# GATECH-EIC/PipeGCN

Hardware: AMD Instinct MI355X
Metric: epoch time (s), reddit 3-layer GraphSAGE (full-graph, pipelined) (lower is better)
Workload: dtype fp32; 1 GPU; model=graphsage-3L-h256, graph=reddit, num_nodes=232965, avg_degree=492, n_feat=602, n_class=41, pipeline=True, use_pp=False, norm=layer, parallelism=graph-partition dp1, num_halo=0, num_edges=114851422

## Files before the change

pipegcn_amd/csrc/bindings.cpp:

```cpp

#include "common.h"

#include <optional>

static torch::Tensor spmm(torch::Tensor indptr, torch::Tensor indices,
                          torch::Tensor feat, torch::Tensor dst_scale,
                          torch::Tensor src_scale, torch::Tensor row_order,
                          int64_t num_rows,
                          std::optional<torch::Tensor> n_live) {
  if (feat.is_cuda()) {
    auto out = torch::empty({num_rows, feat.size(1)}, feat.options());
    spmm_csr_hip(indptr, indices, feat, dst_scale, src_scale, row_order,
                 out, n_live.value_or(torch::Tensor()));
    return out;
  }
  if (feat.scalar_type() == torch::kBFloat16) {
    return spmm_cpu(indptr, indices, feat.to(torch::kFloat), dst_scale,
                    src_scale, num_rows)
        .to(torch::kBFloat16);
  }
  return spmm_cpu(indptr, indices, feat, dst_scale, src_scale, num_rows);
}

static torch::Tensor spmm_drop(torch::Tensor indptr, torch::Tensor indices,
                               torch::Tensor feat, torch::Tensor dst_scale,
                               torch::Tensor src_scale,
                               torch::Tensor row_order, int64_t num_rows,
                               bool transposed, int64_t drop_key,
                               int64_t drop_thr, double drop_scale,
                               std::optional<torch::Tensor> n_live) {
  TORCH_CHECK(feat.is_cuda() && feat.dim() == 2,
              "spmm_drop is the GPU path");
  auto out = torch::empty({num_rows, feat.size(1)}, feat.options());
  spmm_drop_hip(indptr, indices, feat, dst_scale, src_scale, row_order, out,
                n_live.value_or(torch::Tensor()), transposed, drop_key,
                drop_thr, drop_scale);
  return out;
}

static std::vector<torch::Tensor> spmm_max(torch::Tensor indptr,
                                           torch::Tensor indices,
                                           torch::Tensor z,
                                           torch::Tensor row_order,
                                           int64_t num_rows, int64_t num_cols,
                                           bool with_arg) {
  TORCH_CHECK(indptr.numel() == num_rows + 1,
              "spmm_max: indptr must hold num_rows + 1 entries");
  if (z.is_cuda())
// ... 135 lines not shown
}

static std::vector<torch::Tensor> layer_norm_relu_bwd(
    torch::Tensor dy, torch::Tensor xhat, torch::Tensor rstd,
    torch::Tensor w, torch::Tensor b, bool relu) {
  auto dx = torch::empty_like(dy);
  const int64_t N = dy.size(0);
  const int64_t F = dy.size(1);
  const int64_t nblk = std::min<int64_t>(1024, (N + 3) / 4);
  auto dw_part = torch::empty({nblk * 4, F},
                              dy.options().dtype(torch::kFloat));
  auto db_part = torch::empty_like(dw_part);
  layer_norm_relu_bwd_hip(dy.contiguous(), xhat, rstd, w, b, relu, dx,
                          dw_part, db_part);
  return {dx, colsum_hip(dw_part), colsum_hip(db_part)};
}

static void ema_update(torch::Tensor avg, torch::Tensor x, double momentum) {
  if (avg.is_cuda()) {
    ema_update_hip(avg, x, momentum);
  } else {
    avg.mul_(momentum).add_(x, 1.0 - momentum);
  }
}

PYBIND11_MODULE(TORCH_EXTENSION_NAME, m) {
  m.doc() = "pipegcn_amd native core (gfx950 HIP kernels + host graph ops)";
  m.def("build_csr", &build_csr, "COO -> CSR (counting sort by dst)");
  m.def("partition_graph", &partition_graph_cpu,
        "BFS-grown + refined k-way partitioner (cut/vol objective)");
  m.def("spmm", &spmm, "CSR SpMM with fused scale epilogue (fwd & transpose)",
        py::arg("indptr"), py::arg("indices"), py::arg("feat"),
        py::arg("dst_scale"), py::arg("src_scale"), py::arg("row_order"),
        py::arg("num_rows"), py::arg("n_live") = py::none());
  m.def("spmm_drop", &spmm_drop,
        "CSR SpMM over the edges the edge-dropout hash keeps, times "
        "drop_scale",
        py::arg("indptr"), py::arg("indices"), py::arg("feat"),
        py::arg("dst_scale"), py::arg("src_scale"), py::arg("row_order"),
        py::arg("num_rows"), py::arg("transposed"), py::arg("drop_key"),
        py::arg("drop_thr"), py::arg("drop_scale"),
        py::arg("n_live") = py::none());
  m.def("csr_simple", &csr_simple,
        "CSR without repeated entries in a row -> (indptr, indices, removed)");
  m.def("spmm_max", &spmm_max,
        "max aggregation over the CSR -> [out] or [out, arg]",
        py::arg("indptr"), py::arg("indices"), py::arg("z"),
        py::arg("row_order"), py::arg("num_rows"), py::arg("num_cols"),
        py::arg("with_arg"));
  m.def("spmm_max_bwd", &spmm_max_bwd,
        "grad_z of the max aggregation (GPU: over the simple CSC)",
        py::arg("indptr"), py::arg("indices"), py::arg("g"), py::arg("arg"),
        py::arg("row_order"), py::arg("num_src"), py::arg("num_cols"));
  m.def("scale_rows_live", &scale_rows_live,
        "g * inv per row -> (scaled, n_live = 1 + last non-zero row, int32)");
  m.def("pack_rows", &pack_rows,
        "fp32 [N, F] -> packed rows int32 [N, stride_words]");
  m.def("spmm_packed", &spmm_packed,
        "CSR SpMM over packed rows (fp32, dst_scale epilogue)");
  m.def("gather_rows", &gather_rows, "out[i,:] = src[idx[i],:]");
  m.def("gather_rows_out", &gather_rows_out,
        "gather into a preallocated out buffer");
  m.def("scatter_add_rows", &scatter_add_rows, "dst[idx[i],:] += src[i,:]");
  m.def("ema_update", &ema_update, "avg = m*avg + (1-m)*x");
  m.def("colsum", &colsum, "out[n] = sum_m x[m,n]");
  m.def("sage_dual_gemm", &sage_dual_gemm,
        "out = x1 @ w1^T + x2 @ w2^T + bias (MFMA fp32, fused)");
// ... 54 lines not shown
```

pipegcn_amd/csrc/common.h:

```cpp
#pragma once

#include <torch/extension.h>

#include <cstdint>
#include <vector>


std::vector<torch::Tensor> build_csr(torch::Tensor u, torch::Tensor v,
                                     int64_t num_rows);

torch::Tensor partition_graph_cpu(torch::Tensor indptr, torch::Tensor indices,
                                  int64_t nparts, int64_t objective,
                                  double balance_slack, int64_t n_refine_passes,
                                  int64_t seed);

torch::Tensor spmm_cpu(torch::Tensor indptr, torch::Tensor indices,
                       torch::Tensor feat, torch::Tensor dst_scale,
                       torch::Tensor src_scale, int64_t num_rows);

std::vector<torch::Tensor> max_aggregate_cpu(torch::Tensor indptr,
                                             torch::Tensor indices,
                                             torch::Tensor z, int64_t num_rows,
                                             bool with_arg);
torch::Tensor max_aggregate_bwd_cpu(torch::Tensor g, torch::Tensor arg,
                                    int64_t num_src);

std::vector<torch::Tensor> csr_simple(torch::Tensor indptr,
                                      torch::Tensor indices);


int pick_vec(int64_t F, int64_t num_rows, int64_t elem_size = 4);

std::vector<torch::Tensor> spmm_max_fwd_hip(torch::Tensor indptr,
                                            torch::Tensor indices,
                                            torch::Tensor z,
                                            torch::Tensor row_order,
                                            int64_t num_cols, bool with_arg);
torch::Tensor spmm_max_bwd_hip(torch::Tensor indptr, torch::Tensor indices,
                               torch::Tensor g, torch::Tensor arg,
                               torch::Tensor row_order, int64_t num_cols);

void spmm_csr_hip(torch::Tensor indptr, torch::Tensor indices,
                  torch::Tensor feat, torch::Tensor dst_scale,
                  torch::Tensor src_scale, torch::Tensor row_order,
                  torch::Tensor out, torch::Tensor n_live = {});

void scale_rows_live_hip(torch::Tensor g, torch::Tensor inv,
                         torch::Tensor scaled, torch::Tensor n_live);

void spmm_drop_hip(torch::Tensor indptr, torch::Tensor indices,
                   torch::Tensor feat, torch::Tensor dst_scale,
                   torch::Tensor src_scale, torch::Tensor row_order,
                   torch::Tensor out, torch::Tensor n_live, bool transposed,
                   int64_t drop_key, int64_t drop_thr, double drop_scale);

struct PackedLayout {
  int64_t mask_words;
  int64_t hdr_words;
  int64_t stride_words;
};
PackedLayout packed_layout(int64_t F);
void pack_rows_hip(torch::Tensor x, torch::Tensor packed);
void spmm_packed_hip(torch::Tensor indptr, torch::Tensor indices,
                     torch::Tensor packed, int64_t F, torch::Tensor dst_scale,
                     torch::Tensor row_order, torch::Tensor out);

void gather_rows_hip(torch::Tensor src, torch::Tensor idx, torch::Tensor out);

void scatter_add_rows_hip(torch::Tensor dst, torch::Tensor idx,
                          torch::Tensor src);

void ema_update_hip(torch::Tensor avg, torch::Tensor x, double momentum);

torch::Tensor colsum_hip(torch::Tensor x);

void dropout_fwd_hip(torch::Tensor x, torch::Tensor y, torch::Tensor mask,
                     double p, int64_t seed);
void dropout_bwd_hip(torch::Tensor dy, torch::Tensor mask, torch::Tensor dx,
// ... 53 lines not shown
```

pipegcn_amd/csrc/hip/kernels.hip:

```cpp

#include "../common.h"
#include "hip_util.h"

#include <hip/hip_bf16.h>
#include <hip/hip_runtime.h>

#include <cstdlib>
#include <vector>

namespace {

__device__ __forceinline__ void st_nt(float* p, float v) {
  __builtin_nontemporal_store(v, p);
}
__device__ __forceinline__ void st_nt(__hip_bfloat16* p, float v) {
  union {
    __hip_bfloat16 b;
    unsigned short u;
  } cv;
  cv.b = __float2bfloat16(v);
  __builtin_nontemporal_store(cv.u, reinterpret_cast<unsigned short*>(p));
}
__device__ __forceinline__ void st(float* p, float v) { *p = v; }
__device__ __forceinline__ void st(__hip_bfloat16* p, float v) {
  *p = __float2bfloat16(v);
}


template <typename T, int VEC, bool HAS_SRC_SCALE, bool HAS_LIVE>
__global__ void spmm_csr_kernel(const int64_t* __restrict__ indptr,
                                const int32_t* __restrict__ indices,
                                const T* __restrict__ feat,
                                const float* __restrict__ dst_scale,
                                const float* __restrict__ src_scale,
                                const int32_t* __restrict__ row_order,
                                T* __restrict__ out, int64_t num_rows,
                                int64_t F, int64_t nchunks,
                                const int32_t* __restrict__ n_live) {
  static_assert(!(HAS_SRC_SCALE && HAS_LIVE),
                "the redirect would also redirect the scale's index");
  int32_t live = 0;
  if constexpr (HAS_LIVE) live = max(*n_live, 0);
  auto node = [&](int32_t u) -> int64_t {
    return HAS_LIVE ? min(u, live) : u;
  };
  const int wave_in_block =
      __builtin_amdgcn_readfirstlane(static_cast<int>(threadIdx.x) / kWave);
  const int64_t waves_per_block = blockDim.x / kWave;
  const int64_t wave_global =
      static_cast<int64_t>(blockIdx.x) * waves_per_block + wave_in_block;
  const int lane = threadIdx.x & (kWave - 1);
  const int64_t nwaves = static_cast<int64_t>(gridDim.x) * waves_per_block;
  const int64_t npairs = num_rows * nchunks;

  for (int64_t pair = wave_global; pair < npairs; pair += nwaves) {
    int64_t r = pair / nchunks;
    const int64_t chunk = pair % nchunks;
    if (row_order) r = row_order[r];
    const int64_t f0 = chunk * (kWave * VEC) + lane * VEC;
    if (f0 >= F) continue;
    const bool full = (f0 + VEC <= F);

    float acc[VEC];
#pragma unroll
    for (int k = 0; k < VEC; ++k) acc[k] = 0.f;

    const int64_t e_begin = indptr[r];
    const int64_t e_end = indptr[r + 1];
    int64_t e = e_begin;

    if (full) {
// ... 13 lines not shown
        float s0 = 1.f, s1 = 1.f, s2 = 1.f, s3 = 1.f;
        if (HAS_SRC_SCALE) {
          s0 = src_scale[u0];
          s1 = src_scale[u1];
          s2 = src_scale[u2];
          s3 = src_scale[u3];
        }
        float v0[VEC], v1[VEC], v2[VEC], v3[VEC];
#pragma unroll
        for (int k = 0; k < VEC; ++k) v0[k] = to_f32(feat[u0 * F + f0 + k]);
#pragma unroll
        for (int k = 0; k < VEC; ++k) v1[k] = to_f32(feat[u1 * F + f0 + k]);
#pragma unroll
        for (int k = 0; k < VEC; ++k) v2[k] = to_f32(feat[u2 * F + f0 + k]);
#pragma unroll
        for (int k = 0; k < VEC; ++k) v3[k] = to_f32(feat[u3 * F + f0 + k]);
        if (HAS_SRC_SCALE) {
#pragma unroll
          for (int k = 0; k < VEC; ++k)
            acc[k] += s0 * v0[k] + s1 * v1[k] + s2 * v2[k] + s3 * v3[k];
        } else {
#pragma unroll
          for (int k = 0; k < VEC; ++k)
            acc[k] += v0[k] + v1[k] + v2[k] + v3[k];
        }
      }
      for (; e < e_end; ++e) {
        const int64_t u = node(indices[e]);
        const float s = HAS_SRC_SCALE ? src_scale[u] : 1.f;
#pragma unroll
        for (int k = 0; k < VEC; ++k)
          acc[k] += s * to_f32(feat[u * F + f0 + k]);
      }
      const float s = dst_scale ? dst_scale[r] : 1.f;
#pragma unroll
      for (int k = 0; k < VEC; ++k) st_nt(out + r * F + f0 + k, acc[k] * s);
    } else {
      for (; e < e_end; ++e) {
        const int64_t u = node(indices[e]);
        const float s = HAS_SRC_SCALE ? src_scale[u] : 1.f;
        for (int k = 0; k < VEC && f0 + k < F; ++k)
          acc[k] += s * to_f32(feat[u * F + f0 + k]);
      }
      const float s = dst_scale ? dst_scale[r] : 1.f;
      for (int k = 0; k < VEC && f0 + k < F; ++k)
        st(out + r * F + f0 + k, acc[k] * s);
    }
  }
}

template <typename T, int VEC>
void launch_spmm(const int64_t* indptr, const int32_t* indices,
                 const T* feat, const float* dst_scale,
                 const float* src_scale, const int32_t* row_order,
                 const int32_t* n_live, T* out, int64_t num_rows, int64_t F,
                 hipStream_t stream) {
  const int64_t nchunks = (F + kWave * VEC - 1) / (kWave * VEC);
  constexpr int threads = 256;
  static_assert(threads % kWave == 0);
  const int64_t blocks = grid_for(num_rows * nchunks, threads);
  auto launch = [&](auto kern) {
    hipLaunchKernelGGL(kern, dim3(blocks), dim3(threads), 0, stream, indptr,
                       indices, feat, dst_scale, src_scale, row_order, out,
                       num_rows, F, nchunks, n_live);
  };
  if (n_live)
    launch(HIP_KERNEL_NAME(spmm_csr_kernel<T, VEC, false, true>));
  else if (src_scale)
    launch(HIP_KERNEL_NAME(spmm_csr_kernel<T, VEC, true, false>));
  else
    launch(HIP_KERNEL_NAME(spmm_csr_kernel<T, VEC, false, false>));
  check_launch();
}


template <typename T, int VEC, bool SCATTER_ADD>
__global__ void rowcopy_kernel(const T* __restrict__ src,
                               const int64_t* __restrict__ idx,
                               T* __restrict__ dst, int64_t nrows,
                               int64_t F, int64_t nchunks) {
  const int64_t wave_global =
      (static_cast<int64_t>(blockIdx.x) * blockDim.x + threadIdx.x) / kWave;
  const int lane = threadIdx.x & (kWave - 1);
  const int64_t nwaves =
      (static_cast<int64_t>(gridDim.x) * blockDim.x) / kWave;
  const int64_t npairs = nrows * nchunks;
  for (int64_t pair = wave_global; pair < npairs; pair += nwaves) {
    const int64_t i = pair / nchunks;
    const int64_t f0 = pair % nchunks * (kWave * VEC) + lane * VEC;
    if (f0 >= F) continue;
    const int64_t j = idx[i];
    if (f0 + VEC <= F) {
#pragma unroll
      for (int k = 0; k < VEC; ++k) {
        if (SCATTER_ADD)
          st(dst + j * F + f0 + k, to_f32(dst[j * F + f0 + k]) +
                                       to_f32(src[i * F + f0 + k]));
        else
          dst[i * F + f0 + k] = src[j * F + f0 + k];
      }
    } else {
      for (int k = 0; f0 + k < F; ++k) {
        if (SCATTER_ADD)
          st(dst + j * F + f0 + k, to_f32(dst[j * F + f0 + k]) +
// ... 6 lines not shown
}

template <typename T, int VEC, bool SCATTER_ADD>
void launch_rowcopy(const T* src, const int64_t* idx, T* dst,
                    int64_t nrows, int64_t F, hipStream_t stream) {
  const int64_t nchunks = (F + kWave * VEC - 1) / (kWave * VEC);
  const int threads = 256;
  const int64_t blocks = grid_for(nrows * nchunks, threads);
  hipLaunchKernelGGL(HIP_KERNEL_NAME(rowcopy_kernel<T, VEC, SCATTER_ADD>),
                     dim3(blocks), dim3(threads), 0, stream, src, idx, dst,
                     nrows, F, nchunks);
  check_launch();
}


__global__ void ema_kernel(float* __restrict__ avg,
                           const float* __restrict__ x, float m, int64_t n) {
  const int64_t i4 = (static_cast<int64_t>(blockIdx.x) * blockDim.x +
                      threadIdx.x) * 4;
  if (i4 + 4 <= n) {
    float4 a = *reinterpret_cast<float4*>(avg + i4);
    const float4 b = *reinterpret_cast<const float4*>(x + i4);
    a.x = m * a.x + (1.f - m) * b.x;
    a.y = m * a.y + (1.f - m) * b.y;
    a.z = m * a.z + (1.f - m) * b.z;
    a.w = m * a.w + (1.f - m) * b.w;
    *reinterpret_cast<float4*>(avg + i4) = a;
  } else {
    for (int64_t i = i4; i < n; ++i) avg[i] = m * avg[i] + (1.f - m) * x[i];
  }
}


template <int VEC>
__global__ void colsum_partial_kernel(const float* __restrict__ x,
                                      float* __restrict__ partials,
                                      int64_t M, int64_t F,
                                      int64_t rows_per_blk) {
  const int64_t blk = blockIdx.x;
  const int64_t r0 = blk * rows_per_blk;
  const int64_t r1 = min(r0 + rows_per_blk, M);
  for (int64_t f0 = static_cast<int64_t>(threadIdx.x) * VEC; f0 < F;
       f0 += 256 * VEC) {
    float acc[VEC];
#pragma unroll
    for (int k = 0; k < VEC; ++k) acc[k] = 0.f;
    if (f0 + VEC <= F) {
      for (int64_t r = r0; r < r1; ++r) {
#pragma unroll
        for (int k = 0; k < VEC; ++k) acc[k] += x[r * F + f0 + k];
      }
#pragma unroll
      for (int k = 0; k < VEC; ++k) partials[blk * F + f0 + k] = acc[k];
    } else {
      for (int64_t r = r0; r < r1; ++r)
        for (int k = 0; f0 + k < F; ++k) acc[k] += x[r * F + f0 + k];
      for (int k = 0; f0 + k < F; ++k) partials[blk * F + f0 + k] = acc[k];
    }
  }
}

}

int pick_vec(int64_t F, int64_t num_rows, int64_t elem_size) {
  if (const char* e = std::getenv("PIPEGCN_SPMM_VEC")) {
    int v = std::atoi(e);
    if ((v == 8 || v == 4 || v == 2 || v == 1) && F % v == 0 &&
        v * elem_size <= 16)
      return v;
  }
  const bool big = num_rows >= (1 << 20);
  const std::initializer_list<int> pref =
      big ? std::initializer_list<int>{16, 8, 4}
          : std::initializer_list<int>{8, 16, 4};
  for (int bytes : pref) {
    if (bytes < elem_size) continue;
    const int v = bytes / static_cast<int>(elem_size);
    if (F % v == 0) return v;
  }
  return 1;
}

template <typename T>
void spmm_dispatch(torch::Tensor& indptr, torch::Tensor& indices,
                   torch::Tensor& feat, const float* dsp, const float* ssp,
                   const int32_t* rop, const int32_t* nlp, torch::Tensor& out,
                   int64_t num_rows, int64_t F, int vec, hipStream_t stream) {
  const T* fp = reinterpret_cast<const T*>(feat.data_ptr());
  T* op = reinterpret_cast<T*>(out.data_ptr());
  const int64_t* ip = indptr.data_ptr<int64_t>();
  const int32_t* xp = indices.data_ptr<int32_t>();
  dispatch_vec(vec, [&](auto v) {
    launch_spmm<T, v.value>(ip, xp, fp, dsp, ssp, rop, nlp, op, num_rows, F,
                            stream);
  });
}

void spmm_csr_hip(torch::Tensor indptr, torch::Tensor indices,
                  torch::Tensor feat, torch::Tensor dst_scale,
                  torch::Tensor src_scale, torch::Tensor row_order,
                  torch::Tensor out, torch::Tensor n_live) {
  TORCH_CHECK(feat.is_cuda() && out.is_cuda(), "spmm_csr_hip: device tensors");
  const bool bf16 = feat.scalar_type() == torch::kBFloat16;
  TORCH_CHECK(bf16 || feat.scalar_type() == torch::kFloat,
              "spmm: fp32 or bf16 only");
  TORCH_CHECK(out.scalar_type() == feat.scalar_type());
  TORCH_CHECK(feat.is_contiguous() && out.is_contiguous());
  TORCH_CHECK(indptr.scalar_type() == torch::kLong &&
              indices.scalar_type() == torch::kInt);
  const int64_t num_rows = out.size(0);
  const int64_t num_src = feat.size(0);
  const int64_t F = feat.size(1);
  TORCH_CHECK(out.size(1) == F && indptr.numel() == num_rows + 1);
  const float* dsp = nullptr;
  if (dst_scale.defined() && dst_scale.numel() > 0) {
    TORCH_CHECK(dst_scale.is_contiguous() && dst_scale.numel() == num_rows);
    TORCH_CHECK(dst_scale.scalar_type() == torch::kFloat);
    dsp = dst_scale.data_ptr<float>();
  }
  const float* ssp = nullptr;
  if (src_scale.defined() && src_scale.numel() > 0) {
    TORCH_CHECK(src_scale.is_contiguous() && src_scale.numel() == num_src);
    TORCH_CHECK(src_scale.scalar_type() == torch::kFloat);
    ssp = src_scale.data_ptr<float>();
  }
  const int32_t* rop = nullptr;
  if (row_order.defined() && row_order.numel() > 0) {
    TORCH_CHECK(row_order.is_contiguous() && row_order.numel() == num_rows &&
                row_order.scalar_type() == torch::kInt);
    rop = row_order.data_ptr<int32_t>();
  }
  const int32_t* nlp = nullptr;
  if (n_live.defined() && n_live.numel() > 0) {
    TORCH_CHECK(n_live.is_cuda() && n_live.numel() == 1 &&
                    n_live.scalar_type() == torch::kInt,
                "spmm: n_live is one int32 in device memory");
    TORCH_CHECK(ssp == nullptr,
                "spmm: n_live and src_scale do not combine (the redirect "
                "would pick another row's scale)");
    nlp = n_live.data_ptr<int32_t>();
  }
  auto stream = current_stream();
  const int vec = pick_vec(F, num_rows, bf16 ? 2 : 4);
  if (bf16)
    spmm_dispatch<__hip_bfloat16>(indptr, indices, feat, dsp, ssp, rop, nlp,
                                  out, num_rows, F, vec, stream);
  else
    spmm_dispatch<float>(indptr, indices, feat, dsp, ssp, rop, nlp, out,
                         num_rows, F, vec, stream);
}

template <typename T, bool SCATTER_ADD>
void rowcopy_dispatch(torch::Tensor& src, torch::Tensor& idx,
                      torch::Tensor& dst, int64_t n, int64_t F,
                      int vec, hipStream_t stream) {
  const T* sp = reinterpret_cast<const T*>(src.data_ptr());
  T* dp = reinterpret_cast<T*>(dst.data_ptr());
  const int64_t* ixp = idx.data_ptr<int64_t>();
  dispatch_vec(vec, [&](auto v) {
    launch_rowcopy<T, v.value, SCATTER_ADD>(sp, ixp, dp, n, F, stream);
  });
}

void gather_rows_hip(torch::Tensor src, torch::Tensor idx, torch::Tensor out) {
  TORCH_CHECK(src.is_cuda() && idx.is_cuda() && out.is_cuda());
  const bool bf16 = src.scalar_type() == torch::kBFloat16;
  TORCH_CHECK(bf16 || src.scalar_type() == torch::kFloat);
  TORCH_CHECK(out.scalar_type() == src.scalar_type() &&
              idx.scalar_type() == torch::kLong);
  TORCH_CHECK(src.is_contiguous() && out.is_contiguous());
  const int64_t F = src.size(1);
  const int64_t n = idx.numel();
  TORCH_CHECK(out.size(0) == n && out.size(1) == F);
  auto stream = current_stream();
  const int vec = pick_vec(F, 0, bf16 ? 2 : 4);
  if (bf16)
    rowcopy_dispatch<__hip_bfloat16, false>(src, idx, out, n, F, vec, stream);
  else
    rowcopy_dispatch<float, false>(src, idx, out, n, F, vec, stream);
}

// ... 52 lines not shown
```

pipegcn_amd/models/sage.py:

```python
from __future__ import annotations

import math

import torch
from torch import nn

from pipegcn_amd import ops
from pipegcn_amd.graph.csr import FullGraph, HaloGraph
from pipegcn_amd.models.sync_bn import SyncBatchNorm
from pipegcn_amd.parallel import context as ctx


def check_edge_drop(edge_drop):
    if not 0.0 <= edge_drop < 1.0:
        raise ValueError(f"edge_drop={edge_drop} is outside [0, 1)")
    return edge_drop


class GraphSAGELayer(nn.Module):

    def __init__(self, in_feats, out_feats, bias=True, use_pp=False,
                 edge_drop=0.0):
        super().__init__()
        self.use_pp = use_pp
        self.edge_drop = check_edge_drop(edge_drop)
        if use_pp:
            self.linear = nn.Linear(2 * in_feats, out_feats, bias=bias)
        else:
            self.linear1 = nn.Linear(in_feats, out_feats, bias=bias)
            self.linear2 = nn.Linear(in_feats, out_feats, bias=bias)
        self.reset_parameters()

    def reset_parameters(self):
        def init(lin):
            stdv = 1.0 / math.sqrt(lin.weight.size(1))
            lin.weight.data.uniform_(-stdv, stdv)
            if lin.bias is not None:
                lin.bias.data.uniform_(-stdv, stdv)

        if self.use_pp:
            init(self.linear)
        else:
            init(self.linear1)
            init(self.linear2)

    def forward(self, graph, feat, in_deg=None):
        if self.training:
            if self.use_pp:
                return self.linear(feat)
            assert isinstance(graph, HaloGraph)
            inv_deg = (1.0 / in_deg.clamp(min=1.0)).contiguous()
            if self.edge_drop > 0:
                ah = ops.spmm_mean(graph, feat, inv_deg,
                                   edge_drop=self.edge_drop)
            else:
                ah = ops.spmm_mean(graph, feat, inv_deg)
            x1 = feat[: graph.num_in]
            if feat.is_cuda:
                return ops.sage_dual_linear(x1, ah, self.linear1,
                                            self.linear2)
            return self.linear1(x1) + self.linear2(ah)
        assert isinstance(graph, FullGraph) and in_deg is None
        degs = graph.in_degrees().clamp(min=1.0)
        ah = ops.spmm(graph.csr, feat, (1.0 / degs).contiguous())
        if self.use_pp:
            return self.linear(torch.cat((feat, ah), dim=1))
        return self.linear1(feat) + self.linear2(ah)


class SAGEPoolLayer(nn.Module):

    def __init__(self, in_feats, out_feats, bias=True):
        super().__init__()
        self.linear_pool = nn.Linear(in_feats, in_feats, bias=True)
        self.linear1 = nn.Linear(in_feats, out_feats, bias=bias)
        self.linear2 = nn.Linear(in_feats, out_feats, bias=bias)
        self.reset_parameters()

    def reset_parameters(self):
        for lin in (self.linear_pool, self.linear1, self.linear2):
            stdv = 1.0 / math.sqrt(lin.weight.size(1))
            lin.weight.data.uniform_(-stdv, stdv)
            if lin.bias is not None:
                lin.bias.data.uniform_(-stdv, stdv)
# ... 24 lines not shown
        self.n_linear = n_linear
        self.use_norm = norm is not None
        if self.use_norm:
            self.norm = nn.ModuleList()
        self.dropout = nn.Dropout(p=dropout)
        for i in range(self.n_layers):
            if i < self.n_layers - n_linear:
                self.layers.append(self.make_conv(i, layer_size[i],
                                                  layer_size[i + 1], **conv))
            else:
                self.layers.append(nn.Linear(layer_size[i],
                                             layer_size[i + 1]))
            if i < self.n_layers - 1 and self.use_norm:
                if norm == "layer":
                    self.norm.append(
                        nn.LayerNorm(layer_size[i + 1],
                                     elementwise_affine=True))
                elif norm == "batch":
                    self.norm.append(SyncBatchNorm(layer_size[i + 1],
                                                   train_size))

    def make_conv(self, i, in_feats, out_feats, **conv):
        raise NotImplementedError

    def _exchanges_input(self, i):
        return True

    def forward(self, g, feat, in_deg=None):
        h = feat
        for i in range(self.n_layers):
            if i < self.n_layers - self.n_linear:
                if self.training and self._exchanges_input(i):
                    h = ctx.buffer.update(i, h)
                h = self._drop(h)
                h = self.layers[i](g, h, in_deg)
            else:
                h = self._drop(h)
                h = ops.linear(h, self.layers[i])
            if i < self.n_layers - 1:
                h = self._norm_act(i, h)
        return h

    def _drop(self, h):
        if self.training and h.is_cuda and self.dropout.p > 0:
            return ops.fused_dropout(h, self.dropout.p)
        return self.dropout(h)

    def _norm_act(self, i, h):
        if h.is_cuda and self.use_norm and isinstance(self.norm[i],
                                                      nn.LayerNorm):
            fuse_relu = self.activation is torch.nn.functional.relu
            h = ops.layer_norm_relu(h, self.norm[i], relu=fuse_relu)
            return h if fuse_relu else self.activation(h)
        if self.use_norm:
            h = self.norm[i](h)
        return self.activation(h)


AGGREGATORS = ("mean", "pool")


class GraphSAGE(GNNBase):
    def __init__(self, layer_size, activation, use_pp, dropout=0.5,
                 norm="layer", train_size=None, n_linear=0,
                 aggregator="mean", edge_drop=0.0):
        if aggregator not in AGGREGATORS:
            raise ValueError(f"unknown aggregator {aggregator!r}: one of "
                             f"{', '.join(AGGREGATORS)}")
# ... 23 lines not shown
```

pipegcn_amd/ops/__init__.py:

```python
from __future__ import annotations

import math
import os
from typing import Optional

import torch

from pipegcn_amd import native
from pipegcn_amd.graph.csr import CSR, HaloGraph


def _row_order(matrix: CSR) -> torch.Tensor:
    return matrix.row_order if matrix.row_order is not None else torch.Tensor()


def _tune_row_order(csr: CSR, feat, s, ss) -> bool:
    import time

    nat = torch.Tensor()
    times = {}
    for key, ro in (("lpt", csr.row_order), ("nat", nat)):
        native().spmm(csr.indptr, csr.indices, feat, s, ss, ro,
                      csr.num_rows)
        torch.cuda.synchronize()
        t0 = time.perf_counter()
        for _ in range(2):
            native().spmm(csr.indptr, csr.indices, feat, s, ss, ro,
                          csr.num_rows)
        torch.cuda.synchronize()
        times[key] = time.perf_counter() - t0
    return times["lpt"] <= times["nat"]


def spmm(csr: CSR, feat: torch.Tensor,
         scale: Optional[torch.Tensor] = None,
         src_scale: Optional[torch.Tensor] = None,
         n_live: Optional[torch.Tensor] = None) -> torch.Tensor:
    if feat.shape[0] < csr.num_cols:
        raise ValueError(
            f"spmm: feat has {feat.shape[0]} rows but the graph references "
            f"{csr.num_cols} source nodes (an under-sized feat would be an "
            "out-of-bounds GPU gather)")
    s = scale if scale is not None else torch.Tensor()
    ss = src_scale if src_scale is not None else torch.Tensor()
    feat = feat.contiguous()
    ro = _row_order(csr)
    if (feat.is_cuda and csr.row_order is not None
            and csr.nnz * feat.shape[1] >= (1 << 30)
            and os.environ.get("PIPEGCN_SPMM_AUTOTUNE", "1") == "1"):
        cache = getattr(csr, "_lpt_choice", None)
        if cache is None:
            cache = {}
            csr._lpt_choice = cache
        use_lpt = cache.get(feat.shape[1])
        if use_lpt is None:
            free, _ = torch.cuda.mem_get_info(feat.device)
            out_bytes = csr.num_rows * feat.shape[1] * feat.element_size()
            if free < 3 * out_bytes + (2 << 30):
                use_lpt = True
            else:
                use_lpt = _tune_row_order(csr, feat, s, ss)
            cache[feat.shape[1]] = use_lpt
        if not use_lpt:
            ro = torch.Tensor()
    if n_live is None:
        return native().spmm(csr.indptr, csr.indices, feat, s, ss,
                             ro, csr.num_rows)
    return native().spmm(csr.indptr, csr.indices, feat, s, ss,
                         ro, csr.num_rows, n_live)


def scale_rows_live(g: torch.Tensor, inv: torch.Tensor):
    return native().scale_rows_live(g, inv)


def packed_row_layout(F: int):
    mask_words = (F + 31) // 32
    hdr_words = (2 * mask_words + 3) // 4 * 4
    stride_words = (hdr_words + F + 8 + 31) // 32 * 32
    return mask_words, hdr_words, stride_words


def pack_rows_reference(x: torch.Tensor) -> torch.Tensor:
    if x.dim() != 2 or x.dtype != torch.float32:
        raise ValueError("pack_rows_reference: fp32 [N, F] only")
    N, F = x.shape
    W, hdr, stride = packed_row_layout(F)
    nz = x != 0
    nzp = torch.zeros(N, W * 32, dtype=torch.int64, device=x.device)
    nzp[:, :F] = nz
    nzp = nzp.view(N, W, 32)
    mask = (nzp << torch.arange(32, device=x.device)).sum(-1)
    cnt = nzp.sum(-1)
    prefix = cnt.cumsum(-1) - cnt
    out = torch.zeros(N, stride, dtype=torch.int32, device=x.device)
    out[:, 0:2 * W:2] = ((mask + 2 ** 31) % 2 ** 32 - 2 ** 31).int()
    out[:, 1:2 * W:2] = prefix.int()
# ... 28 lines not shown

def _spmm_packed_width(F: int) -> bool:
    return F >= 64


def _spmm_packed_route(feat: torch.Tensor) -> bool:
    if (not feat.is_cuda or feat.dtype != torch.float32
            or os.environ.get("PIPEGCN_SPMM_PACKED", "1") == "0"
            or not _spmm_packed_width(feat.shape[1])):
        return False
    free, _ = torch.cuda.mem_get_info(feat.device)
    need = feat.shape[0] * packed_row_layout(feat.shape[1])[2] * 4
    return free >= need + (2 << 30)


def spmm_packed(csr: CSR, feat: torch.Tensor,
                scale: Optional[torch.Tensor] = None) -> torch.Tensor:
    if feat.shape[0] < csr.num_cols:
        raise ValueError(
            f"spmm_packed: feat has {feat.shape[0]} rows but the graph "
            f"references {csr.num_cols} source nodes (an under-sized feat "
            "would be an out-of-bounds GPU gather)")
    if not feat.is_cuda or feat.dtype != torch.float32 or feat.dim() != 2:
        raise ValueError("spmm_packed: fp32 [N, F] GPU tensors only")
    s = scale if scale is not None else torch.Tensor()
    ro = _row_order(csr)
    if getattr(csr, "_lpt_choice", {}).get(feat.shape[1]) is False:
        ro = torch.Tensor()
    packed = native().pack_rows(feat.contiguous())
    return native().spmm_packed(csr.indptr, csr.indices, packed,
                                feat.shape[1], s, ro, csr.num_rows)


class _SpmmMean(torch.autograd.Function):

    @staticmethod
    def forward(ctx, graph: HaloGraph, feat: torch.Tensor,
                inv_deg: torch.Tensor):
        ctx.graph = graph
        ctx.save_for_backward(inv_deg)
        if _spmm_packed_route(feat):
            return spmm_packed(graph.csr, feat, inv_deg)
        return spmm(graph.csr, feat, inv_deg)

    @staticmethod
    def backward(ctx, grad_out: torch.Tensor):
        (inv_deg,) = ctx.saved_tensors
        g = ctx.graph
        if g.csc.nnz > grad_out.numel():
            if grad_out.is_cuda:
                scaled, n_live = scale_rows_live(grad_out, inv_deg)
                if os.environ.get("PIPEGCN_SPMM_LIVE", "1") == "0":
                    n_live = None
                grad_feat = spmm(g.csc, scaled, None, n_live=n_live)
            else:
                grad_feat = spmm(
                    g.csc,
                    grad_out * inv_deg.unsqueeze(1).to(grad_out.dtype), None)
        else:
            grad_feat = spmm(g.csc, grad_out.contiguous(), None,
                             src_scale=inv_deg)
        return None, grad_feat, None


class _SpmmMeanDrop(torch.autograd.Function):

    @staticmethod
    def forward(ctx, graph: HaloGraph, feat: torch.Tensor,
                inv_deg: torch.Tensor, drop):
        ctx.graph, ctx.drop = graph, drop
        ctx.save_for_backward(inv_deg)
        return spmm_drop(graph.csr, feat, inv_deg, drop=drop)

    @staticmethod
    def backward(ctx, grad_out: torch.Tensor):
        (inv_deg,) = ctx.saved_tensors
        g, drop = ctx.graph, ctx.drop
        if g.csc.nnz > grad_out.numel():
            n_live = None
            if grad_out.is_cuda:
                scaled, n_live = scale_rows_live(grad_out, inv_deg)
                if os.environ.get("PIPEGCN_SPMM_LIVE", "1") == "0":
                    n_live = None
            else:
                scaled = grad_out * inv_deg.unsqueeze(1).to(grad_out.dtype)
            grad_feat = spmm_drop(g.csc, scaled, drop=drop, transposed=True,
                                  n_live=n_live)
        else:
            grad_feat = spmm_drop(g.csc, grad_out.contiguous(),
                                  src_scale=inv_deg, drop=drop,
                                  transposed=True)
        return None, grad_feat, None, None


def spmm_mean(graph: HaloGraph, feat: torch.Tensor, inv_deg: torch.Tensor,
# ... 421 lines not shown
    return _BiasColsum.apply(x, b)


def gather_rows(src: torch.Tensor, idx: torch.Tensor) -> torch.Tensor:
    return native().gather_rows(src.contiguous(), idx)


def gather_rows_into(src: torch.Tensor, idx: torch.Tensor,
                     out: torch.Tensor) -> None:
    if src.is_cuda:
        native().gather_rows_out(src.contiguous(), idx, out)
    else:
        torch.index_select(src, 0, idx, out=out)


def scatter_add_rows(dst: torch.Tensor, idx: torch.Tensor,
                     src: torch.Tensor) -> None:
    native().scatter_add_rows(dst, idx, src.contiguous())


def ema_update(avg: torch.Tensor, x: torch.Tensor, momentum: float) -> None:
    if avg.dtype != torch.float32:
        avg.mul_(momentum).add_(x, alpha=1.0 - momentum)
        return
    native().ema_update(avg, x, momentum)


class _SageDualLinear(torch.autograd.Function):

    @staticmethod
    def forward(ctx, x1, x2, w1, w2, b1, b2):
        ctx.save_for_backward(x1, x2, w1, w2)
        ctx.has_bias = b1 is not None
        if (w1.size(0) < 64 or not x1.is_cuda
                or x1.dtype != torch.float32):
            out = torch.mm(x1, w1.t())
            out.addmm_(x2, w2.t())
            if b1 is not None:
                out.add_(b1 + b2)
            return out
        bias = (b1 + b2) if b1 is not None else torch.Tensor()
        return native().sage_dual_gemm(x1.contiguous(), x2.contiguous(),
                                       w1.contiguous(), w2.contiguous(),
                                       bias)

    @staticmethod
    def backward(ctx, g):
        x1, x2, w1, w2 = ctx.saved_tensors
        g = g.contiguous()
        if g.is_cuda and g.dtype == torch.float32:
            gw1, gw2 = native().dual_wgrad(g, x1.contiguous(),
                                           x2.contiguous())
            if g.size(1) >= 64 and w1.size(1) <= 256:
                gx1, gx2 = native().dual_dgrad(g, w1.contiguous(),
                                               w2.contiguous())
            else:
                gx = g @ torch.cat((w1, w2), dim=1)
                K = w1.size(1)
                gx1, gx2 = gx[:, :K], gx[:, K:]
        else:
            gx1 = g @ w1
            gx2 = g @ w2
            gw1 = g.t() @ x1
            gw2 = g.t() @ x2
        if not ctx.has_bias:
            return gx1, gx2, gw1, gw2, None, None
        gb = native().colsum(g)
        gb = gb.to(w1.dtype)
        return gx1, gx2, gw1, gw2, gb, gb


def sage_dual_linear(x1, x2, lin1, lin2):
    return _SageDualLinear.apply(x1, x2, lin1.weight, lin2.weight, lin1.bias,
                                 lin2.bias)


class _FusedDropout(torch.autograd.Function):

    @staticmethod
    def forward(ctx, x, p, seed):
        y, mask = native().dropout_fwd(x.contiguous(), p, seed)
        ctx.save_for_backward(mask)
        ctx.p = p
        return y

    @staticmethod
    def backward(ctx, dy):
        (mask,) = ctx.saved_tensors
        return native().dropout_bwd(dy, mask, ctx.p), None, None


def fused_dropout(x: torch.Tensor, p: float) -> torch.Tensor:
    seed = int(torch.randint(0, 2 ** 62, (1,)).item())
    return _FusedDropout.apply(x, p, seed)


class _LayerNormReLU(torch.autograd.Function):

    @staticmethod
    def forward(ctx, x, w, b, eps, relu):
        y, xhat, rstd = native().layer_norm_relu_fwd(
            x.contiguous(), w.contiguous(), b.contiguous(), eps, relu)
# ... 4 lines not shown
    @staticmethod
    def backward(ctx, dy):
        xhat, rstd, w, b = ctx.saved_tensors
        dx, dw, db = native().layer_norm_relu_bwd(dy, xhat, rstd, w, b,
                                                  ctx.relu)
        return dx, dw, db, None, None


def layer_norm_relu(x: torch.Tensor, ln: torch.nn.LayerNorm,
                    relu: bool) -> torch.Tensor:
    return _LayerNormReLU.apply(x, ln.weight.float(), ln.bias.float(),
                                ln.eps, relu)


class _LinearColsum(torch.autograd.Function):

    @staticmethod
    def forward(ctx, x, w, b):
        ctx.save_for_backward(x, w)
        out = torch.mm(x, w.t())
        if b is not None:
            out.add_(b)
        return out

    @staticmethod
    def backward(ctx, g):
        x, w = ctx.saved_tensors
        g = g.contiguous()
        gb = native().colsum(g).to(w.dtype)
        if g.dtype == torch.float32:
            (gw,) = native().dual_wgrad(g, x.contiguous(), torch.Tensor())
        else:
            gw = g.t() @ x
        return g @ w, gw, gb


def linear(x, lin):
    if not x.is_cuda or lin.bias is None:
        return lin(x)
    return _LinearColsum.apply(x, lin.weight, lin.bias)
```

Baseline: 0.07752 s/epoch.

## Fuse SAGE layer backward: residual add and dropout mask into SpMM epilogue

```diff
diff --git a/pipegcn_amd/csrc/bindings.cpp b/pipegcn_amd/csrc/bindings.cpp
--- a/pipegcn_amd/csrc/bindings.cpp
+++ b/pipegcn_amd/csrc/bindings.cpp
@@ -7,13 +7,21 @@
                           torch::Tensor feat, torch::Tensor dst_scale,
                           torch::Tensor src_scale, torch::Tensor row_order,
                           int64_t num_rows,
-                          std::optional<torch::Tensor> n_live) {
+                          std::optional<torch::Tensor> n_live,
+                          std::optional<torch::Tensor> add_rows,
+                          int64_t n_add,
+                          std::optional<torch::Tensor> drop_mask,
+                          double drop_scale) {
   if (feat.is_cuda()) {
     auto out = torch::empty({num_rows, feat.size(1)}, feat.options());
     spmm_csr_hip(indptr, indices, feat, dst_scale, src_scale, row_order,
-                 out, n_live.value_or(torch::Tensor()));
+                 out, n_live.value_or(torch::Tensor()),
+                 add_rows.value_or(torch::Tensor()), n_add,
+                 drop_mask.value_or(torch::Tensor()), drop_scale);
     return out;
   }
+  TORCH_CHECK(!add_rows.has_value() && !drop_mask.has_value(),
+              "spmm: the add/dropout epilogue is the GPU path");
   if (feat.scalar_type() == torch::kBFloat16) {
     return spmm_cpu(indptr, indices, feat.to(torch::kFloat), dst_scale,
                     src_scale, num_rows)
@@ -215,7 +223,9 @@
   m.def("spmm", &spmm, "CSR SpMM with fused scale epilogue (fwd & transpose)",
         py::arg("indptr"), py::arg("indices"), py::arg("feat"),
         py::arg("dst_scale"), py::arg("src_scale"), py::arg("row_order"),
-        py::arg("num_rows"), py::arg("n_live") = py::none());
+        py::arg("num_rows"), py::arg("n_live") = py::none(),
+        py::arg("add_rows") = py::none(), py::arg("n_add") = 0,
+        py::arg("drop_mask") = py::none(), py::arg("drop_scale") = 1.0);
   m.def("spmm_drop", &spmm_drop,
         "CSR SpMM over the edges the edge-dropout hash keeps, times "
         "drop_scale",
diff --git a/pipegcn_amd/csrc/common.h b/pipegcn_amd/csrc/common.h
--- a/pipegcn_amd/csrc/common.h
+++ b/pipegcn_amd/csrc/common.h
@@ -43,7 +43,9 @@
 void spmm_csr_hip(torch::Tensor indptr, torch::Tensor indices,
                   torch::Tensor feat, torch::Tensor dst_scale,
                   torch::Tensor src_scale, torch::Tensor row_order,
-                  torch::Tensor out, torch::Tensor n_live = {});
+                  torch::Tensor out, torch::Tensor n_live = {},
+                  torch::Tensor add_rows = {}, int64_t n_add = 0,
+                  torch::Tensor drop_mask = {}, double drop_scale = 1.0);
 
 void scale_rows_live_hip(torch::Tensor g, torch::Tensor inv,
                          torch::Tensor scaled, torch::Tensor n_live);
diff --git a/pipegcn_amd/csrc/hip/kernels.hip b/pipegcn_amd/csrc/hip/kernels.hip
--- a/pipegcn_amd/csrc/hip/kernels.hip
+++ b/pipegcn_amd/csrc/hip/kernels.hip
@@ -26,8 +26,41 @@
   *p = __float2bfloat16(v);
 }
 
-
-template <typename T, int VEC, bool HAS_SRC_SCALE, bool HAS_LIVE>
+__device__ __forceinline__ float rounded(float v, const float*) { return v; }
+__device__ __forceinline__ float rounded(float v, const __hip_bfloat16*) {
+  return __bfloat162float(__float2bfloat16(v));
+}
+
+
+struct SpmmEpilogue {
+  const void* add_rows;
+  int64_t add_stride;
+  int64_t n_add;
+  const uint8_t* drop_mask;
+  float drop_scale;
+};
+
+template <typename T>
+__device__ __forceinline__ float spmm_epilogue(const SpmmEpilogue& ep,
+                                               float acc, int64_t r,
+                                               int64_t c, int64_t F) {
+  const T* tag = nullptr;
+  float v = rounded(acc, tag);
+  if (ep.add_rows != nullptr) {
+    const float a = r < ep.n_add ? to_f32(static_cast<const T*>(
+                                       ep.add_rows)[r * ep.add_stride + c])
+                                 : 0.f;
+    v = rounded(v + a, tag);
+  }
+  if (ep.drop_mask != nullptr) {
+    const int64_t i = r * F + c;
+    const bool keep = (ep.drop_mask[i >> 3] >> (i & 7)) & 1;
+    v = keep ? rounded(v * ep.drop_scale, tag) : 0.f;
+  }
+  return v;
+}
+
+template <typename T, int VEC, bool HAS_SRC_SCALE, bool HAS_LIVE, bool EPI>
 __global__ void spmm_csr_kernel(const int64_t* __restrict__ indptr,
                                 const int32_t* __restrict__ indices,
                                 const T* __restrict__ feat,
@@ -36,7 +69,8 @@
                                 const int32_t* __restrict__ row_order,
                                 T* __restrict__ out, int64_t num_rows,
                                 int64_t F, int64_t nchunks,
-                                const int32_t* __restrict__ n_live) {
+                                const int32_t* __restrict__ n_live,
+                                SpmmEpilogue ep) {
   static_assert(!(HAS_SRC_SCALE && HAS_LIVE),
                 "the redirect would also redirect the scale's index");
   int32_t live = 0;
@@ -116,9 +150,16 @@
         for (int k = 0; k < VEC; ++k)
           acc[k] += s * to_f32(feat[u * F + f0 + k]);
       }
-      const float s = dst_scale ? dst_scale[r] : 1.f;
-#pragma unroll
-      for (int k = 0; k < VEC; ++k) st_nt(out + r * F + f0 + k, acc[k] * s);
+      if constexpr (EPI) {
+#pragma unroll
+        for (int k = 0; k < VEC; ++k)
+          st_nt(out + r * F + f0 + k,
+                spmm_epilogue<T>(ep, acc[k], r, f0 + k, F));
+      } else {
+        const float s = dst_scale ? dst_scale[r] : 1.f;
+#pragma unroll
+        for (int k = 0; k < VEC; ++k) st_nt(out + r * F + f0 + k, acc[k] * s);
+      }
     } else {
       for (; e < e_end; ++e) {
         const int64_t u = node(indices[e]);
@@ -126,9 +167,15 @@
         for (int k = 0; k < VEC && f0 + k < F; ++k)
           acc[k] += s * to_f32(feat[u * F + f0 + k]);
       }
-      const float s = dst_scale ? dst_scale[r] : 1.f;
-      for (int k = 0; k < VEC && f0 + k < F; ++k)
-        st(out + r * F + f0 + k, acc[k] * s);
+      if constexpr (EPI) {
+        for (int k = 0; k < VEC && f0 + k < F; ++k)
+          st(out + r * F + f0 + k,
+             spmm_epilogue<T>(ep, acc[k], r, f0 + k, F));
+      } else {
+        const float s = dst_scale ? dst_scale[r] : 1.f;
+        for (int k = 0; k < VEC && f0 + k < F; ++k)
+          st(out + r * F + f0 + k, acc[k] * s);
+      }
     }
   }
 }
@@ -137,8 +184,8 @@
 void launch_spmm(const int64_t* indptr, const int32_t* indices,
                  const T* feat, const float* dst_scale,
                  const float* src_scale, const int32_t* row_order,
-                 const int32_t* n_live, T* out, int64_t num_rows, int64_t F,
-                 hipStream_t stream) {
+                 const int32_t* n_live, const SpmmEpilogue* epi, T* out,
+                 int64_t num_rows, int64_t F, hipStream_t stream) {
   const int64_t nchunks = (F + kWave * VEC - 1) / (kWave * VEC);
   constexpr int threads = 256;
   static_assert(threads % kWave == 0);
@@ -146,14 +193,23 @@
   auto launch = [&](auto kern) {
     hipLaunchKernelGGL(kern, dim3(blocks), dim3(threads), 0, stream, indptr,
                        indices, feat, dst_scale, src_scale, row_order, out,
-                       num_rows, F, nchunks, n_live);
+                       num_rows, F, nchunks, n_live,
+                       epi ? *epi : SpmmEpilogue{});
   };
-  if (n_live)
-    launch(HIP_KERNEL_NAME(spmm_csr_kernel<T, VEC, false, true>));
-  else if (src_scale)
-    launch(HIP_KERNEL_NAME(spmm_csr_kernel<T, VEC, true, false>));
-  else
-    launch(HIP_KERNEL_NAME(spmm_csr_kernel<T, VEC, false, false>));
+  if (epi) {
+    if (n_live)
+      launch(HIP_KERNEL_NAME(spmm_csr_kernel<T, VEC, false, true, true>));
+    else if (src_scale)
+      launch(HIP_KERNEL_NAME(spmm_csr_kernel<T, VEC, true, false, true>));
+    else
+      launch(HIP_KERNEL_NAME(spmm_csr_kernel<T, VEC, false, false, true>));
+  } else if (n_live) {
+    launch(HIP_KERNEL_NAME(spmm_csr_kernel<T, VEC, false, true, false>));
+  } else if (src_scale) {
+    launch(HIP_KERNEL_NAME(spmm_csr_kernel<T, VEC, true, false, false>));
+  } else {
+    launch(HIP_KERNEL_NAME(spmm_csr_kernel<T, VEC, false, false, false>));
+  }
   check_launch();
 }
 
@@ -226,6 +282,8 @@
 }
 
 
+constexpr int kColsumRows = 16;
+
 template <int VEC>
 __global__ void colsum_partial_kernel(const float* __restrict__ x,
                                       float* __restrict__ partials,
@@ -240,7 +298,19 @@
 #pragma unroll
     for (int k = 0; k < VEC; ++k) acc[k] = 0.f;
     if (f0 + VEC <= F) {
-      for (int64_t r = r0; r < r1; ++r) {
+      int64_t r = r0;
+      for (; r + kColsumRows <= r1; r += kColsumRows) {
+        float v[kColsumRows][VEC];
+#pragma unroll
+        for (int j = 0; j < kColsumRows; ++j)
+#pragma unroll
+          for (int k = 0; k < VEC; ++k) v[j][k] = x[(r + j) * F + f0 + k];
+#pragma unroll
+        for (int j = 0; j < kColsumRows; ++j)
+#pragma unroll
+          for (int k = 0; k < VEC; ++k) acc[k] += v[j][k];
+      }
+      for (; r < r1; ++r) {
 #pragma unroll
         for (int k = 0; k < VEC; ++k) acc[k] += x[r * F + f0 + k];
       }
@@ -278,22 +348,25 @@
 template <typename T>
 void spmm_dispatch(torch::Tensor& indptr, torch::Tensor& indices,
                    torch::Tensor& feat, const float* dsp, const float* ssp,
-                   const int32_t* rop, const int32_t* nlp, torch::Tensor& out,
+                   const int32_t* rop, const int32_t* nlp,
+                   const SpmmEpilogue* epi, torch::Tensor& out,
                    int64_t num_rows, int64_t F, int vec, hipStream_t stream) {
   const T* fp = reinterpret_cast<const T*>(feat.data_ptr());
   T* op = reinterpret_cast<T*>(out.data_ptr());
   const int64_t* ip = indptr.data_ptr<int64_t>();
   const int32_t* xp = indices.data_ptr<int32_t>();
   dispatch_vec(vec, [&](auto v) {
-    launch_spmm<T, v.value>(ip, xp, fp, dsp, ssp, rop, nlp, op, num_rows, F,
-                            stream);
+    launch_spmm<T, v.value>(ip, xp, fp, dsp, ssp, rop, nlp, epi, op, num_rows,
+                            F, stream);
   });
 }
 
 void spmm_csr_hip(torch::Tensor indptr, torch::Tensor indices,
                   torch::Tensor feat, torch::Tensor dst_scale,
                   torch::Tensor src_scale, torch::Tensor row_order,
-                  torch::Tensor out, torch::Tensor n_live) {
+                  torch::Tensor out, torch::Tensor n_live,
+                  torch::Tensor add_rows, int64_t n_add,
+                  torch::Tensor drop_mask, double drop_scale) {
   TORCH_CHECK(feat.is_cuda() && out.is_cuda(), "spmm_csr_hip: device tensors");
   const bool bf16 = feat.scalar_type() == torch::kBFloat16;
   TORCH_CHECK(bf16 || feat.scalar_type() == torch::kFloat,
@@ -334,13 +407,42 @@
                 "would pick another row's scale)");
     nlp = n_live.data_ptr<int32_t>();
   }
+  SpmmEpilogue ep{};
+  if (add_rows.defined() && add_rows.numel() > 0) {
+    TORCH_CHECK(add_rows.is_cuda() && add_rows.dim() == 2 &&
+                    add_rows.scalar_type() == feat.scalar_type() &&
+                    add_rows.size(1) == F &&
+                    (F == 1 || add_rows.stride(1) == 1),
+                "spmm: add_rows is [n_add, F] in feat's dtype, rows "
+                "contiguous");
+    TORCH_CHECK(n_add >= 0 && n_add <= add_rows.size(0),
+                "spmm: n_add exceeds add_rows");
+    TORCH_CHECK(add_rows.size(0) <= 1 || add_rows.stride(0) >= F,
+                "spmm: add_rows rows overlap");
+    ep.add_rows = add_rows.data_ptr();
+    ep.add_stride = add_rows.stride(0);
+    ep.n_add = n_add;
+  }
+  if (drop_mask.defined() && drop_mask.numel() > 0) {
+    TORCH_CHECK(drop_mask.is_cuda() && drop_mask.is_contiguous() &&
+                    drop_mask.scalar_type() == torch::kUInt8 &&
+                    drop_mask.numel() >= (num_rows * F + 7) / 8,
+                "spmm: drop_mask holds one bit per output element (uint8)");
+    ep.drop_mask = drop_mask.data_ptr<uint8_t>();
+    ep.drop_scale = static_cast<float>(drop_scale);
+  }
+  const bool has_epi = ep.add_rows != nullptr || ep.drop_mask != nullptr;
+  TORCH_CHECK(!(has_epi && dsp != nullptr),
+              "spmm: the add/dropout epilogue and dst_scale do not combine "
+              "(acc * scale + add would round once)");
+  const SpmmEpilogue* epi = has_epi ? &ep : nullptr;
   auto stream = current_stream();
   const int vec = pick_vec(F, num_rows, bf16 ? 2 : 4);
   if (bf16)
     spmm_dispatch<__hip_bfloat16>(indptr, indices, feat, dsp, ssp, rop, nlp,
-                                  out, num_rows, F, vec, stream);
+                                  epi, out, num_rows, F, vec, stream);
   else
-    spmm_dispatch<float>(indptr, indices, feat, dsp, ssp, rop, nlp, out,
+    spmm_dispatch<float>(indptr, indices, feat, dsp, ssp, rop, nlp, epi, out,
                          num_rows, F, vec, stream);
 }
 
diff --git a/pipegcn_amd/models/sage.py b/pipegcn_amd/models/sage.py
--- a/pipegcn_amd/models/sage.py
+++ b/pipegcn_amd/models/sage.py
@@ -1,6 +1,7 @@
 from __future__ import annotations
 
 import math
+import os
 
 import torch
 from torch import nn
@@ -44,12 +45,28 @@
             init(self.linear1)
             init(self.linear2)
 
-    def forward(self, graph, feat, in_deg=None):
+    def _can_fuse(self, feat):
+        return (self.training and not self.use_pp and self.edge_drop == 0
+                and feat.is_cuda)
+
+    def fuses_dropout(self, feat):
+        return (self._can_fuse(feat)
+                and os.environ.get("PIPEGCN_SAGE_FUSED", "1") != "0")
+
+    def forward(self, graph, feat, in_deg=None, dropout=None):
+        if dropout is not None and not self._can_fuse(feat):
+            raise ValueError("GraphSAGELayer: only the fused training path "
+                             "(GPU, mean aggregation, no edge dropout, not "
+                             "use_pp) applies feature dropout itself")
         if self.training:
             if self.use_pp:
                 return self.linear(feat)
             assert isinstance(graph, HaloGraph)
             inv_deg = (1.0 / in_deg.clamp(min=1.0)).contiguous()
+            if dropout is not None:
+                return ops.sage_mean_layer(graph, feat, inv_deg,
+                                           self.linear1, self.linear2,
+                                           p=dropout)
             if self.edge_drop > 0:
                 ah = ops.spmm_mean(graph, feat, inv_deg,
                                    edge_drop=self.edge_drop)
@@ -140,8 +157,13 @@
             if i < self.n_layers - self.n_linear:
                 if self.training and self._exchanges_input(i):
                     h = ctx.buffer.update(i, h)
-                h = self._drop(h)
-                h = self.layers[i](g, h, in_deg)
+                layer = self.layers[i]
+                if (isinstance(layer, GraphSAGELayer)
+                        and layer.fuses_dropout(h)):
+                    h = layer(g, h, in_deg, dropout=self.dropout.p)
+                else:
+                    h = self._drop(h)
+                    h = layer(g, h, in_deg)
             else:
                 h = self._drop(h)
                 h = ops.linear(h, self.layers[i])
diff --git a/pipegcn_amd/ops/__init__.py b/pipegcn_amd/ops/__init__.py
--- a/pipegcn_amd/ops/__init__.py
+++ b/pipegcn_amd/ops/__init__.py
@@ -32,10 +32,19 @@
     return times["lpt"] <= times["nat"]
 
 
+def dropout_scale(p: float) -> float:
+    p16 = int(p * 65536.0 + 0.5)
+    return (torch.tensor(1.0) / torch.tensor(1.0 - p16 / 65536.0)).item()
+
+
 def spmm(csr: CSR, feat: torch.Tensor,
          scale: Optional[torch.Tensor] = None,
          src_scale: Optional[torch.Tensor] = None,
-         n_live: Optional[torch.Tensor] = None) -> torch.Tensor:
+         n_live: Optional[torch.Tensor] = None, *,
+         add_rows: Optional[torch.Tensor] = None,
+         n_add: Optional[int] = None,
+         drop_mask: Optional[torch.Tensor] = None,
+         drop_scale: float = 1.0) -> torch.Tensor:
     if feat.shape[0] < csr.num_cols:
         raise ValueError(
             f"spmm: feat has {feat.shape[0]} rows but the graph references "
@@ -63,6 +72,18 @@
             cache[feat.shape[1]] = use_lpt
         if not use_lpt:
             ro = torch.Tensor()
+    if add_rows is not None or drop_mask is not None:
+        if scale is not None:
+            raise ValueError(
+                "spmm: the add/dropout epilogue does not combine with scale "
+                "(acc * scale + add would contract to one rounding)")
+        if not feat.is_cuda:
+            raise ValueError("spmm: the add/dropout epilogue is the GPU path")
+        if add_rows is not None and n_add is None:
+            n_add = add_rows.shape[0]
+        return native().spmm(csr.indptr, csr.indices, feat, s, ss, ro,
+                             csr.num_rows, n_live, add_rows, n_add or 0,
+                             drop_mask, drop_scale)
     if n_live is None:
         return native().spmm(csr.indptr, csr.indices, feat, s, ss,
                              ro, csr.num_rows)
@@ -157,6 +178,28 @@
                                 feat.shape[1], s, ro, csr.num_rows)
 
 
+def _spmm_mean_forward(graph: HaloGraph, feat: torch.Tensor,
+                       inv_deg: torch.Tensor) -> torch.Tensor:
+    if _spmm_packed_route(feat):
+        return spmm_packed(graph.csr, feat, inv_deg)
+    return spmm(graph.csr, feat, inv_deg)
+
+
+def _spmm_mean_backward(g: HaloGraph, grad_out: torch.Tensor,
+                        inv_deg: torch.Tensor, **epilogue) -> torch.Tensor:
+    if g.csc.nnz > grad_out.numel():
+        if grad_out.is_cuda:
+            scaled, n_live = scale_rows_live(grad_out, inv_deg)
+            if os.environ.get("PIPEGCN_SPMM_LIVE", "1") == "0":
+                n_live = None
+            return spmm(g.csc, scaled, None, n_live=n_live, **epilogue)
+        return spmm(g.csc,
+                    grad_out * inv_deg.unsqueeze(1).to(grad_out.dtype), None,
+                    **epilogue)
+    return spmm(g.csc, grad_out.contiguous(), None, src_scale=inv_deg,
+                **epilogue)
+
+
 class _SpmmMean(torch.autograd.Function):
 
     @staticmethod
@@ -164,28 +207,12 @@
                 inv_deg: torch.Tensor):
         ctx.graph = graph
         ctx.save_for_backward(inv_deg)
-        if _spmm_packed_route(feat):
-            return spmm_packed(graph.csr, feat, inv_deg)
-        return spmm(graph.csr, feat, inv_deg)
+        return _spmm_mean_forward(graph, feat, inv_deg)
 
     @staticmethod
     def backward(ctx, grad_out: torch.Tensor):
         (inv_deg,) = ctx.saved_tensors
-        g = ctx.graph
-        if g.csc.nnz > grad_out.numel():
-            if grad_out.is_cuda:
-                scaled, n_live = scale_rows_live(grad_out, inv_deg)
-                if os.environ.get("PIPEGCN_SPMM_LIVE", "1") == "0":
-                    n_live = None
-                grad_feat = spmm(g.csc, scaled, None, n_live=n_live)
-            else:
-                grad_feat = spmm(
-                    g.csc,
-                    grad_out * inv_deg.unsqueeze(1).to(grad_out.dtype), None)
-        else:
-            grad_feat = spmm(g.csc, grad_out.contiguous(), None,
-                             src_scale=inv_deg)
-        return None, grad_feat, None
+        return None, _spmm_mean_backward(ctx.graph, grad_out, inv_deg), None
 
 
 class _SpmmMeanDrop(torch.autograd.Function):
@@ -673,42 +700,113 @@
     def forward(ctx, x1, x2, w1, w2, b1, b2):
         ctx.save_for_backward(x1, x2, w1, w2)
         ctx.has_bias = b1 is not None
-        if (w1.size(0) < 64 or not x1.is_cuda
-                or x1.dtype != torch.float32):
-            out = torch.mm(x1, w1.t())
-            out.addmm_(x2, w2.t())
-            if b1 is not None:
-                out.add_(b1 + b2)
-            return out
-        bias = (b1 + b2) if b1 is not None else torch.Tensor()
-        return native().sage_dual_gemm(x1.contiguous(), x2.contiguous(),
-                                       w1.contiguous(), w2.contiguous(),
-                                       bias)
+        return _sage_dual_forward(x1, x2, w1, w2, b1, b2)
 
     @staticmethod
     def backward(ctx, g):
         x1, x2, w1, w2 = ctx.saved_tensors
         g = g.contiguous()
-        if g.is_cuda and g.dtype == torch.float32:
-            gw1, gw2 = native().dual_wgrad(g, x1.contiguous(),
-                                           x2.contiguous())
-            if g.size(1) >= 64 and w1.size(1) <= 256:
-                gx1, gx2 = native().dual_dgrad(g, w1.contiguous(),
-                                               w2.contiguous())
-            else:
-                gx = g @ torch.cat((w1, w2), dim=1)
-                K = w1.size(1)
-                gx1, gx2 = gx[:, :K], gx[:, K:]
-        else:
-            gx1 = g @ w1
-            gx2 = g @ w2
-            gw1 = g.t() @ x1
-            gw2 = g.t() @ x2
-        if not ctx.has_bias:
-            return gx1, gx2, gw1, gw2, None, None
-        gb = native().colsum(g)
-        gb = gb.to(w1.dtype)
+        gw1, gw2, gb = _sage_param_grads(g, x1, x2, w1, ctx.has_bias)
+        gx1 = gx2 = None
+        if ctx.needs_input_grad[0] or ctx.needs_input_grad[1]:
+            gx1, gx2 = _sage_dgrad(g, w1, w2, ctx.needs_input_grad[0],
+                                   ctx.needs_input_grad[1])
         return gx1, gx2, gw1, gw2, gb, gb
+
+
+def _sage_dual_forward(x1, x2, w1, w2, b1, b2):
+    if (w1.size(0) < 64 or not x1.is_cuda
+            or x1.dtype != torch.float32):
+        out = torch.mm(x1, w1.t())
+        out.addmm_(x2, w2.t())
+        if b1 is not None:
+            out.add_(b1 + b2)
+        return out
+    bias = (b1 + b2) if b1 is not None else torch.Tensor()
+    return native().sage_dual_gemm(x1.contiguous(), x2.contiguous(),
+                                   w1.contiguous(), w2.contiguous(),
+                                   bias)
+
+
+def _sage_param_grads(g, x1, x2, w1, has_bias):
+    if g.is_cuda and g.dtype == torch.float32:
+        gw1, gw2 = native().dual_wgrad(g, x1.contiguous(), x2.contiguous())
+    else:
+        gw1 = g.t() @ x1
+        gw2 = g.t() @ x2
+    if not has_bias:
+        return gw1, gw2, None
+    gb = native().colsum(g)
+    return gw1, gw2, gb.to(w1.dtype)
+
+
+def _mm_dgrad(g, w):
+    return g @ w
+
+
+def _sage_dgrad(g, w1, w2, need1=True, need2=True):
+    if g.is_cuda and g.dtype == torch.float32:
+        if g.size(1) >= 64 and w1.size(1) <= 256:
+            gx1, gx2 = native().dual_dgrad(g, w1.contiguous(),
+                                           w2.contiguous())
+            return (gx1 if need1 else None), (gx2 if need2 else None)
+        if need1 and need2:
+            gx = _mm_dgrad(g, torch.cat((w1, w2), dim=1))
+            K = w1.size(1)
+            return gx[:, :K], gx[:, K:]
+    return (_mm_dgrad(g, w1) if need1 else None,
+            _mm_dgrad(g, w2) if need2 else None)
+
+
+class _SageMeanLayer(torch.autograd.Function):
+
+    @staticmethod
+    def forward(ctx, graph: HaloGraph, h, inv_deg, w1, w2, b1, b2, p):
+        mask = None
+        feat = h
+        if p > 0:
+            seed = int(torch.randint(0, 2 ** 62, (1,)).item())
+            feat, mask = native().dropout_fwd(h.contiguous(), p, seed)
+        ah = _spmm_mean_forward(graph, feat, inv_deg)
+        x1 = feat[: graph.num_in]
+        ctx.graph, ctx.p, ctx.has_bias = graph, p, b1 is not None
+        ctx.acts = (ah,) if mask is None else (ah, x1)
+        ctx.save_for_backward(w1, w2, inv_deg, mask,
+                              *((x1,) if mask is None else ()))
+        return _sage_dual_forward(x1, ah, w1, w2, b1, b2)
+
+    @staticmethod
+    def backward(ctx, g):
+        w1, w2, inv_deg, mask, *saved_x1 = ctx.saved_tensors
+        if ctx.acts is None:
+            raise RuntimeError("sage_mean_layer: its activations are freed "
+                               "by the first backward; a second one through "
+                               "a retained graph is not supported")
+        ah, x1 = ctx.acts + tuple(saved_x1)
+        ctx.acts = None
+        g = g.contiguous()
+        gw1, gw2, gb = _sage_param_grads(g, x1, ah, w1, ctx.has_bias)
+        del ah, x1, saved_x1
+        gh = None
+        if ctx.needs_input_grad[1]:
+            gx1, gx2 = _sage_dgrad(g, w1, w2)
+            epilogue = dict(add_rows=gx1, n_add=ctx.graph.num_in)
+            if mask is not None:
+                epilogue.update(drop_mask=mask,
+                                drop_scale=dropout_scale(ctx.p))
+            gh = _spmm_mean_backward(ctx.graph, gx2, inv_deg, **epilogue)
+        return None, gh, None, gw1, gw2, gb, gb, None
+
+
+def sage_mean_layer(graph: HaloGraph, h: torch.Tensor,
+                    inv_deg: torch.Tensor, lin1, lin2,
+                    p: float = 0.0) -> torch.Tensor:
+    if not h.is_cuda:
+        raise ValueError("sage_mean_layer is the GPU path")
+    if not 0.0 <= p < 1.0:
+        raise ValueError(f"sage_mean_layer: p={p} is outside [0, 1)")
+    return _SageMeanLayer.apply(graph, h, inv_deg, lin1.weight, lin2.weight,
+                                lin1.bias, lin2.bias, p)
 
 
 def sage_dual_linear(x1, x2, lin1, lin2):
@@ -779,7 +877,8 @@
             (gw,) = native().dual_wgrad(g, x.contiguous(), torch.Tensor())
         else:
             gw = g.t() @ x
-        return g @ w, gw, gb
+        gx = _mm_dgrad(g, w) if ctx.needs_input_grad[0] else None
+        return gx, gw, gb
 
 
 def linear(x, lin):
```

After: 0.07487 s/epoch, median of 6. 1.04x faster.
